# Wangshihu12/colmap-pcd

Measured on AMD Instinct MI355X. Metric: NN queries/sec + BA-iter ms, 10M-pt cloud / 1M 3D feats, higher is better.
Workload: dtype f32 (NN distances) / f64 (association, BA); 1 GPU; M: 10000000-pt 'planes' cloud / 1000000 queries + BA scene 1000 cams / 1000000 pts / 4721253 obs / 900000 lidar terms (OPENCV), the same total at every N; cloud_points=10000000, queries=1000000, queries_this_rank=1000000, parallelism=single GPU

## Files before the change

colmap-pcd_amd/csrc/brick_clip_kernel.h:

```cpp
#pragma once

namespace pcd {

constexpr int kClipNk = 7;
constexpr int kClipRows = 9;
constexpr int kATile = 128;
constexpr int kClipRanges = 10;
#ifdef PCD_ABLATE
constexpr int kAblateClipMath = 0x10000, kAblateBound = 0x20000, kAblateStageA = 0x40000, kAblateSelect = 0x80000;
#else
constexpr int kAblateClipMath = 0, kAblateBound = 0, kAblateStageA = 0, kAblateSelect = 0;
#endif

__device__ __forceinline__ void compare_q1p1(const f32x4 p, const float qx, const float qy, const float qz, double& best) {
  asm("v_mov_b32 v120, %[pw]\n\t"
      "v_sub_f32 v122, %[qx], %[px]\n\tv_sub_f32 v123, %[qy], %[py]\n\tv_sub_f32 v124, %[qz], %[pz]\n\t"
      "v_mul_f32 v122, v122, v122\n\tv_mul_f32 v123, v123, v123\n\tv_mul_f32 v124, v124, v124\n\t"
      "v_add_f32 v122, v122, v123\n\tv_add_f32 v121, v122, v124\n\t"
      "v_min_f64 %[b], %[b], v[120:121]\n\t"
      : [b] "+v"(best)
      : [px] "v"(p.x), [py] "v"(p.y), [pz] "v"(p.z), [pw] "v"(p.w), [qx] "v"(qx), [qy] "v"(qy), [qz] "v"(qz)
      : "v118", "v119", "v120", "v121", "v122", "v123", "v124", "v125", "v126", "v127");
}

template <int NQ, int NP>
__device__ __forceinline__ void compare_step(const f32x4 (&p)[2], const float (&qx)[8], const float (&qy)[8],
                                             const float (&qz)[8], double (&best)[8]) {
  static_assert(NQ >= 1 && NQ <= 8 && (NP == 1 || NP == 2), "1..8 queries, 1 or 2 points");
  constexpr int E = NQ & ~1;
#pragma unroll
  for (int k = 0; k < NP; ++k) {
    if (E >= 4) compare_point4(p[k], qx, qy, qz, best);
    if (E == 8) compare_point4(p[k], qx + 4, qy + 4, qz + 4, best + 4);
    if (E == 2 || E == 6) compare_point2(p[k], qx + (E - 2), qy + (E - 2), qz + (E - 2), best + (E - 2));
  }
  if (NQ & 1) {
    if (NP == 2) compare_query1(p[0], p[1], qx[NQ - 1], qy[NQ - 1], qz[NQ - 1], best[NQ - 1]);
    else compare_q1p1(p[0], qx[NQ - 1], qy[NQ - 1], qz[NQ - 1], best[NQ - 1]);
  }
}

__device__ __forceinline__ float proven_bound_f(const GridParams& g, float qx, float qy, float qz, const int c0[3],
                                                const int c1[3]) {
  const float q[3] = {qx, qy, qz};
  float margin = 3e38f;
#pragma unroll
  for (int d = 0; d < 3; ++d) {
    if (c0[d] > 0) margin = fminf(margin, q[d] - (g.origin[d] + (float)c0[d] * g.h));
    if (c1[d] < g.dims[d]) margin = fminf(margin, (g.origin[d] + (float)c1[d] * g.h) - q[d]);
  }
  if (margin >= 3e38f) return 3e38f;
  margin -= 2.0f * g.slack;
  if (!(margin > 0.0f)) return -1.0f;
  return margin * margin * (1.0f - 1e-5f);
}

constexpr uint64_t span_lanes(int cls) {
  uint64_t m = 0;
  for (int r = 0; r < kClipRows; ++r)
    for (int j = 0; j < 3; ++j)
      if ((j != 1) + (r % 3 != 1) + (r / 3 != 1) == cls) m |= 1ull << (kClipNk * r + 2 * j);
  return m;
}

struct ClipMeta {
  float4 q;
  uint64_t prior;
  uint32_t bnd;
};

__device__ __forceinline__ ClipMeta clip_load_meta(const GridParams& g, const uint4 it, const float4* __restrict__ qsorted,
                                                   const uint64_t* __restrict__ ksorted,
                                                   const uint32_t* __restrict__ cell_start, uint32_t lpos) {
  const int lane = threadIdx.x & 63;
  const int lk = (int)(lpos & 0xFFu), lry = (int)((lpos >> 8) & 0xFFu), lrz = (int)(lpos >> 16);
  ClipMeta m;
  const int cnt = item_count(it);
  m.q = qsorted[it.x + (lane < cnt ? lane : cnt - 1)];
  m.prior = ksorted[it.x + (lane < cnt ? lane : cnt - 1)];
  const int bx = (int)it.y, by = (int)it.z, bz = (int)(it.w & 0x0FFFFFFFu);
  const int yq = by - 1 + lry, zq = bz - 1 + lrz;
  const bool ok = lrz < 3 && yq >= 0 && yq < g.qdims[0] && zq >= 0 && zq < g.qdims[1];
  const int x = min(max(2 * bx - 2 + lk, 0), g.dims[0]);
  const uint32_t v = cell_start[quad_row_base(g, ok ? yq : 0, ok ? zq : 0) + 4u * (uint64_t)x];
  m.bnd = ok ? v : 0u;
  return m;
}

__global__ __launch_bounds__(256, 4) void k_nn_brick_clip(GridParams g, const float4* __restrict__ sorted,
                                                          const uint32_t* __restrict__ cell_start,
                                                          const float4* __restrict__ qsorted,
                                                          const uint64_t* __restrict__ ksorted,
                                                          const uint4* __restrict__ items, NnCounters* __restrict__ ctr,
                                                          uint64_t* __restrict__ keys, uint32_t* __restrict__ fb_list,
                                                          uint32_t* __restrict__ fb_count, int flags) {
  constexpr int G = 8;
  constexpr int NK = kClipNk, NC = kClipNk - 1;
  const int collect_stats = flags & 1;
  const bool no_clip = (flags & 2) != 0;
  __shared__ __attribute__((aligned(16))) float4 s_tile[4][2][kTile];
  __shared__ __attribute__((aligned(16))) float4 s_a[4][kATile];
  const int lane = threadIdx.x & 63;
  const int wave = __builtin_amdgcn_readfirstlane((int)(threadIdx.x >> 6));
  const uint32_t nitems = ctr->nitems;
  const uint32_t nwaves = gridDim.x * 4;
  unsigned long long st_staged = 0, st_pairs = 0, st_groups = 0;
  uint32_t fb_base = 0, fb_left = 0;
  uint32_t lpos;
  {
    const int lrow = (lane * 9363) >> 16, lk = lane - 7 * lrow;
    const int lrz = (lrow * 21846) >> 16, lry = lrow - 3 * lrz;
    lpos = (uint32_t)lk | ((uint32_t)lry << 8) | ((uint32_t)lrz << 16);
    asm volatile("" : "+v"(lpos));
  }
#define PCD_BND(m, e) PCD_RL((m).bnd, (e))

  uint32_t item, item_end, stride;
  if ((gridDim.x & 7u) == 0) {
    const uint32_t cls = blockIdx.x & 7u, per = (nitems + 7u) / 8u;
    stride = (gridDim.x >> 3) * 4;
    item = cls * per + (blockIdx.x >> 3) * 4 + wave;
    item_end = min(nitems, (cls + 1) * per);
  } else {
    stride = nwaves;
    item = blockIdx.x * 4 + wave;
    item_end = nitems;
  }
  if (item >= item_end) return;
  const char* __restrict__ src_bytes = reinterpret_cast<const char*>(sorted);
  float4* const bufA = s_a[wave];
#define PCD_RL(v, r) ((uint32_t)__builtin_amdgcn_readlane((int)(v), (int)(r)))
  struct ARange { uint32_t s, ne; };
  auto issue_a = [&](const ClipMeta& m) -> ARange {
    uint32_t sA = PCD_BND(m, 4 * NK + 2), eA = PCD_BND(m, 4 * NK + 4);
    uint32_t e = 4 * NK + 2;
    if (sA == eA) {
      uint32_t up = (uint32_t)__builtin_amdgcn_update_dpp((int)m.bnd, (int)m.bnd, 0x130, 0xf, 0xf, false);
      up = (uint32_t)__builtin_amdgcn_update_dpp((int)up, (int)up, 0x130, 0xf, 0xf, false);
      const uint32_t size = up - m.bnd;
      const uint64_t occ = __builtin_amdgcn_ballot_w64(size != 0u);
      const uint64_t fc = occ & span_lanes(1), ed = occ & span_lanes(2), co = occ & span_lanes(3);
      const uint64_t pick = fc ? fc : ed ? ed : co;
      if (pick & (pick - 1)) {
        uint32_t key = ((0xFFFFFFu - min(size, 0xFFFFFFu)) << 6) | (uint32_t)lane;
        asm("v_cndmask_b32_e64 %0, -1, %1, %2" : "=v"(key) : "v"(key), "s"(pick));
        e = wave_min_u32(key) & 63u;
      } else if (pick) {
        e = (uint32_t)__builtin_ctzll(pick);
      }
      sA = PCD_RL(m.bnd, e); eA = PCD_RL(m.bnd, e + 2u);
    }
    const uint32_t nA = min(eA - sA, (uint32_t)kATile);
    const uint32_t last = nA ? nA - 1u : 0u;
    const uint32_t i0 = sA + min((uint32_t)lane, last), i1 = sA + min((uint32_t)lane + 64u, last);
    lds_dma16(reinterpret_cast<const float4*>(src_bytes + ((uint64_t)i0 << 4)), bufA);
    lds_dma16(reinterpret_cast<const float4*>(src_bytes + ((uint64_t)i1 << 4)), bufA + 64);
    return ARange{sA, nA | (e << 8)};
  };

  uint4 it0 = items[PCD_UNI(item)];
  ClipMeta m0 = clip_load_meta(g, it0, qsorted, ksorted, cell_start, lpos);
  uint4 it1 = items[PCD_UNI(min(item + stride, item_end - 1))];
  ARange a0 = issue_a(m0);

  for (; item < item_end; item += stride) {
    asm volatile("s_waitcnt vmcnt(0)" ::: "memory");
    __builtin_amdgcn_wave_barrier();
    const ClipMeta m1 = clip_load_meta(g, it1, qsorted, ksorted, cell_start, lpos);
    const uint4 it2 = items[PCD_UNI(min(item + 2 * stride, item_end - 1))];

    const uint32_t cnt = (uint32_t)item_count(it0);
    float qx[G], qy[G], qz[G];
    {
      typedef float f32x3 __attribute__((ext_vector_type(3)));
      const uint32_t qb = lds_addr(s_tile[wave][0]);
      const f32x4 qrec = {m0.q.x, m0.q.y, m0.q.z, m0.q.w};
      f32x3 qv[G];
      asm volatile("ds_write_b128 %9, %8\n\ts_waitcnt lgkmcnt(0)\n\t"
                   "ds_read_b96 %0, %10\n\tds_read_b96 %1, %10 offset:16\n\tds_read_b96 %2, %10 offset:32\n\t"
                   "ds_read_b96 %3, %10 offset:48\n\tds_read_b96 %4, %10 offset:64\n\tds_read_b96 %5, %10 offset:80\n\t"
                   "ds_read_b96 %6, %10 offset:96\n\tds_read_b96 %7, %10 offset:112\n\ts_waitcnt lgkmcnt(0)"
                   : "=&v"(qv[0]), "=&v"(qv[1]), "=&v"(qv[2]), "=&v"(qv[3]), "=&v"(qv[4]), "=&v"(qv[5]), "=&v"(qv[6]), "=&v"(qv[7])
                   : "v"(qrec), "v"(qb + (uint32_t)lane * 16u), "v"(qb)
                   : "memory");
#pragma unroll
      for (int k = 0; k < G; ++k) { qx[k] = qv[k].x; qy[k] = qv[k].y; qz[k] = qv[k].z; }
    }
    const int bx = (int)it0.y, by = (int)it0.z, bz = (int)(it0.w & 0x0FFFFFFFu);
    double best[G];
#pragma unroll
    for (int k = 0; k < G; ++k) best[k] = __builtin_bit_cast(double, kKeyInit);

    const uint32_t sA = a0.s, nA = a0.ne & 0xFFu;
    if (nA > 0 && !(flags & kAblateStageA)) {
      f32x4 pa[2];
      const uint32_t rd = lds_addr(bufA) + lane * 16;
      asm volatile("ds_read_b128 %0, %2\n\tds_read_b128 %1, %2 offset:1024\n\ts_waitcnt lgkmcnt(0)"
                   : "=&v"(pa[0]), "=&v"(pa[1]) : "v"(rd) : "memory");
      if (flags & kAblateCompare) {
        asm volatile("" ::"v"(pa[0]), "v"(pa[1]));
      } else if (nA > 64) {
        switch (cnt) {
          case 1: compare_step<1, 2>(pa, qx, qy, qz, best); break;
          case 2: compare_step<2, 2>(pa, qx, qy, qz, best); break;
          case 3: compare_step<3, 2>(pa, qx, qy, qz, best); break;
          case 4: compare_step<4, 2>(pa, qx, qy, qz, best); break;
          case 5: compare_step<5, 2>(pa, qx, qy, qz, best); break;
          case 6: compare_step<6, 2>(pa, qx, qy, qz, best); break;
          case 7: compare_step<7, 2>(pa, qx, qy, qz, best); break;
          default: compare_step<8, 2>(pa, qx, qy, qz, best); break;
        }
      } else {
        switch (cnt) {
          case 1: compare_step<1, 1>(pa, qx, qy, qz, best); break;
          case 2: compare_step<2, 1>(pa, qx, qy, qz, best); break;
          case 3: compare_step<3, 1>(pa, qx, qy, qz, best); break;
          case 4: compare_step<4, 1>(pa, qx, qy, qz, best); break;
          case 5: compare_step<5, 1>(pa, qx, qy, qz, best); break;
          case 6: compare_step<6, 1>(pa, qx, qy, qz, best); break;
          case 7: compare_step<7, 1>(pa, qx, qy, qz, best); break;
          default: compare_step<8, 1>(pa, qx, qy, qz, best); break;
        }
      }
    }
    const int holder = ((lane & 4) ? 32 : 0) | ((lane & 2) ? 16 : 0) | ((lane & 1) ? 8 : 0);
    uint64_t mine;
    {
      const uint64_t red = __builtin_bit_cast(uint64_t, (flags & kAblateReduce) ? best[0] : wave_min8_key(best));
      mine = ((uint64_t)__shfl((uint32_t)(red >> 32), holder) << 32) | __shfl((uint32_t)red, holder);
      mine = min_u64(mine, m0.prior);
    }
    uint32_t w0 = 0, w1 = 0, w2 = 0;
    if (flags & kAblateClipMath) {
      w0 = w1 = w2 = lane < (int)cnt ? 0x3FFFFu : 0u;
    } else if (lane < (int)cnt) {
      const float d = __uint_as_float((uint32_t)(mine >> 32));
      const float r = __builtin_amdgcn_sqrtf(d) * 1.00001f + ((fabsf(m0.q.x) + fabsf(m0.q.y)) + fabsf(m0.q.z)) * 2.4e-7f + 1e-18f;
      const float tx0 = floorf((m0.q.x - r - g.origin[0]) * g.inv_h), tx1 = floorf((m0.q.x + r - g.origin[0]) * g.inv_h);
      const float ty0 = floorf((m0.q.y - r - g.origin[1]) * g.inv_h * 0.5f), ty1 = floorf((m0.q.y + r - g.origin[1]) * g.inv_h * 0.5f);
      const float tz0 = floorf((m0.q.z - r - g.origin[2]) * g.inv_h * 0.5f), tz1 = floorf((m0.q.z + r - g.origin[2]) * g.inv_h * 0.5f);
      const float fx = (float)(2 * bx - 2), fy = (float)(by - 1), fz = (float)(bz - 1);
      const uint32_t kx0 = (uint32_t)__builtin_amdgcn_fmed3f(tx0 - fx, 0.f, (float)(NC - 1)), kx1 = (uint32_t)__builtin_amdgcn_fmed3f(tx1 - fx, 0.f, (float)(NC - 1));
      const uint32_t ry0 = (uint32_t)__builtin_amdgcn_fmed3f(ty0 - fy, 0.f, 2.f), ry1 = (uint32_t)__builtin_amdgcn_fmed3f(ty1 - fy, 0.f, 2.f);
      const uint32_t rz0 = (uint32_t)__builtin_amdgcn_fmed3f(tz0 - fz, 0.f, 2.f), rz1 = (uint32_t)__builtin_amdgcn_fmed3f(tz1 - fz, 0.f, 2.f);
      const uint32_t xm = (2u << kx1) - (1u << kx0);
      const uint32_t ym = (2u << ry1) - (1u << ry0), zm = (2u << rz1) - (1u << rz0);
      const uint32_t pat = xm * ((ym * 0x421u) & 0x1041u);
      w0 = (zm & 1u) ? pat : 0u; w1 = (zm & 2u) ? pat : 0u; w2 = (zm & 4u) ? pat : 0u;
      if (no_clip) w0 = w1 = w2 = 0x3FFFFu;
    }
#define PCD_OR_SHR(v, ctrl) v |= (uint32_t)__builtin_amdgcn_update_dpp(0, (int)(v), ctrl, 0xf, 0xf, true)
    PCD_OR_SHR(w0, 0x111); PCD_OR_SHR(w1, 0x111); PCD_OR_SHR(w2, 0x111);
    PCD_OR_SHR(w0, 0x112); PCD_OR_SHR(w1, 0x112); PCD_OR_SHR(w2, 0x112);
    PCD_OR_SHR(w0, 0x114); PCD_OR_SHR(w1, 0x114); PCD_OR_SHR(w2, 0x114);
#undef PCD_OR_SHR
    const uint32_t M[3] = {PCD_RL(w0, 7), PCD_RL(w1, 7), PCD_RL(w2, 7)};
    const uint32_t rowA = ((a0.ne >> 8) * 9363u) >> 16;
    const uint32_t bndL = (uint32_t)lane - 7u * rowA < 7u ? min(m0.bnd, sA) : m0.bnd;
    uint32_t rs[kClipRanges], rl[kClipRanges];
#pragma unroll
    for (int r = 0; r < kClipRows; ++r) {
      const uint32_t xm = (M[r / 3] >> (6 * (r % 3))) & 63u;
      const int k0 = xm ? __builtin_ctz(xm) : 0, k1 = xm ? 32 - __builtin_clz(xm) : 0;
      const uint32_t s = PCD_RL(bndL, r * NK + k0), e = PCD_RL(bndL, r * NK + k1);
      rs[r] = s; rl[r] = e - s;
    }
    {
      const uint64_t m54 = (uint64_t)M[0] | ((uint64_t)M[1] << 18) | ((uint64_t)M[2] << 36);
      const uint32_t xm = (uint32_t)(m54 >> (6u * rowA)) & 63u;
      const uint32_t k0 = xm ? (uint32_t)__builtin_ctz(xm) : 0u, k1 = xm ? 32u - (uint32_t)__builtin_clz(xm) : 0u;
      const uint32_t e = PCD_BND(m0, rowA * NK + k1);
      rs[9] = max(PCD_BND(m0, rowA * NK + k0), sA + nA);
      rl[9] = e > rs[9] ? e - rs[9] : 0u;
    }
    uint32_t ro[kClipRanges + 1];
    ro[0] = 0;
#pragma unroll
    for (int i = 0; i < kClipRanges; ++i) ro[i + 1] = ro[i] + ((rl[i] + 3u) & ~3u);
    const uint32_t T = (flags & kAblateTiles) ? 0u : ro[kClipRanges];
    const int ntiles = (int)((T + kTile - 1) / kTile);

    ARange a1;
    if (T > 0) {
      uint32_t dv[kClipRanges];
#pragma unroll
      for (int i = 0; i < kClipRanges; ++i) asm volatile("v_mov_b32 %0, %1" : "=v"(dv[i]) : "s"(rs[i] - ro[i]));
      auto issue_tile = [&](int t) {
        float4* buf = s_tile[wave][t & 1];
        const uint32_t s4 = min((uint32_t)t * kTile + 4u * (uint32_t)lane, T - 4u);
        uint32_t dl = dv[0];
        if (!(flags & kAblateSelect)) {
#define PCD_SEL(o, d) asm("v_cmp_le_u32_e32 vcc, %2, %1\n\tv_cndmask_b32_e32 %0, %0, %3, vcc" : "+v"(dl) : "v"(s4), "s"(o), "v"(d) : "vcc")
        PCD_SEL(ro[1], dv[1]); PCD_SEL(ro[2], dv[2]); PCD_SEL(ro[3], dv[3]); PCD_SEL(ro[4], dv[4]); PCD_SEL(ro[5], dv[5]);
        PCD_SEL(ro[6], dv[6]); PCD_SEL(ro[7], dv[7]); PCD_SEL(ro[8], dv[8]); PCD_SEL(ro[9], dv[9]);
#undef PCD_SEL
        }
        const float4* gp = reinterpret_cast<const float4*>(src_bytes + ((uint64_t)(s4 + dl) << 4));
        if (flags & kAblateNoDma) { asm volatile("" ::"v"(gp)); return; }
        lds_dma16_off<0>(gp, buf);
        lds_dma16_off<16>(gp, buf + 64 - 1);
        lds_dma16_off<32>(gp, buf + 128 - 2);
        lds_dma16_off<48>(gp, buf + 192 - 3);
      };
      issue_tile(0);
      a1 = issue_a(m1);
      auto run_tiles = [&](auto nq_tag) {
        constexpr int NQ = decltype(nq_tag)::value;
        for (int t = 0; t < ntiles; ++t) {
          if (t + 1 < ntiles) {
            issue_tile(t + 1);
            if (t == 0) asm volatile("s_waitcnt vmcnt(6)" ::: "memory");
            else asm volatile("s_waitcnt vmcnt(4)" ::: "memory");
          } else {
            if (t == 0) asm volatile("s_waitcnt vmcnt(2)" ::: "memory");
            else asm volatile("s_waitcnt vmcnt(0)" ::: "memory");
          }
          __builtin_amdgcn_wave_barrier();
          f32x4 p[4];
          const uint32_t rd = lds_addr(s_tile[wave][t & 1]) + lane * 16;
          if (flags & kAblateNoLdsRead) {
#pragma unroll
            for (int k = 0; k < 4; ++k) p[k] = f32x4{(float)lane, (float)t, (float)k, 0.f};
          } else
          asm volatile("ds_read_b128 %0, %4\n\tds_read_b128 %1, %4 offset:1024\n\t"
                       "ds_read_b128 %2, %4 offset:2048\n\tds_read_b128 %3, %4 offset:3072\n\t"
                       "s_waitcnt lgkmcnt(0)"
                       : "=&v"(p[0]), "=&v"(p[1]), "=&v"(p[2]), "=&v"(p[3])
                       : "v"(rd)
                       : "memory");
          if (flags & kAblateCompare) {
#pragma unroll
            for (int k = 0; k < 4; ++k) asm volatile("" ::"v"(p[k]));
          } else {
            compare_tile<NQ>(p, qx, qy, qz, best);
          }
        }
      };
      switch (cnt) {
        case 1: run_tiles(std::integral_constant<int, 1>{}); break;
        case 2: run_tiles(std::integral_constant<int, 2>{}); break;
        case 3: run_tiles(std::integral_constant<int, 3>{}); break;
        case 4: run_tiles(std::integral_constant<int, 4>{}); break;
        case 5: run_tiles(std::integral_constant<int, 5>{}); break;
        case 6: run_tiles(std::integral_constant<int, 6>{}); break;
        case 7: run_tiles(std::integral_constant<int, 7>{}); break;
        default: run_tiles(std::integral_constant<int, 8>{}); break;
      }
      const uint64_t red = __builtin_bit_cast(uint64_t, (flags & kAblateReduce) ? best[0] : wave_min8_key(best));
      mine = min_u64(mine, ((uint64_t)__shfl((uint32_t)(red >> 32), holder) << 32) | __shfl((uint32_t)red, holder));
    } else {
      a1 = issue_a(m1);
    }
    bool unproven = false;
    if (lane < (int)cnt) {
      const uint32_t my_qi = __float_as_uint(m0.q.w);
      const int c0[3] = {max(2 * bx - 2, 0), max(2 * by - 2, 0), max(2 * bz - 2, 0)};
      const int c1[3] = {min(2 * bx + 4, g.dims[0]), min(2 * by + 4, g.dims[1]), min(2 * bz + 4, g.dims[2])};
      const float bound = (flags & kAblateBound) ? 3e38f : proven_bound_f(g, m0.q.x, m0.q.y, m0.q.z, c0, c1);
      unproven = !(__uint_as_float((uint32_t)(mine >> 32)) < bound) && !(flags & kAblateFallback);
      keys[my_qi] = unproven ? mine : finalized_key(mine);
    }
    const unsigned long long um = __ballot(unproven);
    if (um) {
      const uint32_t k = (uint32_t)__popcll(um);
      if (k > fb_left) {
        if (lane < (int)fb_left) fb_list[fb_base + lane] = 0xFFFFFFFFu;
        uint32_t nb = 0;
        if (lane == 0) nb = atomicAdd(fb_count, (uint32_t)kFbChunk);
        fb_base = (uint32_t)__builtin_amdgcn_readfirstlane((int)nb);
        fb_left = kFbChunk;
      }
      if (unproven) fb_list[fb_base + __builtin_amdgcn_mbcnt_hi((uint32_t)(um >> 32), __builtin_amdgcn_mbcnt_lo((uint32_t)um, 0u))] = __float_as_uint(m0.q.w);
      fb_base += k;
      fb_left -= k;
    }
    if (collect_stats) {
      const uint32_t slots = (nA > 64 ? 128u : nA ? 64u : 0u) + (uint32_t)ntiles * kTile;
      st_staged += nA + T; st_pairs += (unsigned long long)slots * cnt; st_groups += 1;
    }
    it0 = it1; it1 = it2; m0 = m1; a0 = a1;
  }
  asm volatile("s_waitcnt vmcnt(0)" ::: "memory");
  if (lane < (int)fb_left) fb_list[fb_base + lane] = 0xFFFFFFFFu;
  if (collect_stats && lane == 0) {
    atomicAdd(&ctr->staged_points, st_staged);
    atomicAdd(&ctr->pair_evals, st_pairs);
    atomicAdd(&ctr->brick_groups, st_groups);
  }
#undef PCD_BND
#undef PCD_RL
}

}
```

colmap-pcd_amd/csrc/nn.hip:

```cpp
#include <atomic>
#include <cfloat>

#include "cloud.h"
#include "grid.h"
#include "prim.h"
#include "scratch.h"

namespace pcd {

void free_query_scratch(QueryScratch* s) { delete s; }

constexpr uint64_t kKeyInit = (uint64_t)0x7F7FFFFFu << 32;
constexpr uint64_t kSmallBatch = 65536;

struct BrickParams {
  int B, R;
  int Bx;
  int nb[3];
  uint32_t nbricks;
};

constexpr int kBrickCells = 2, kBrickCellsX = 2, kBrickHalo = 2;

static BrickParams make_bricks(const GridParams& g) {
// ... 631 lines not shown
      const uint32_t cn_ = (cn);                                                                                      \
      const uint32_t last = cn_ ? cn_ - 1u : 0u;                   \
      const uint32_t id = (cf) + ((uint32_t)lane < last ? (uint32_t)lane : last);                                     \
      const float4 lo = *reinterpret_cast<const float4*>(aabb + 8 * (size_t)id);             \
      const float4 hi = *reinterpret_cast<const float4*>(aabb + 8 * (size_t)id + 4);       \
           \
                      \
      const float px = __builtin_amdgcn_fmed3f(qx, lo.x, lo.w), pyc = __builtin_amdgcn_fmed3f(qy, lo.y, hi.x),        \
                  pz = __builtin_amdgcn_fmed3f(qz, lo.z, hi.y);                                                       \
      const float lbv = l2_simple3(qx, qy, qz, px, pyc, pz);                                                          \
      cur_lb = (uint32_t)lane < cn_ ? lbv : INFINITY;                                                                 \
      rs = __float_as_uint(hi.z); rn = __float_as_uint(hi.w);                                                         \
      cur_m = __ballot(cur_lb <= best_d);                                                                             \
    }
    PCD_FB_EXPAND(py.root_first, py.root_count);
    while (true) {
      ++q_steps;
      unsigned long long m = cur_m & __ballot(cur_lb <= best_d);
      if (m == 0) {
        if (lev == top) break;
        ++lev;
        cur_lb = s_lb[wave][lev - 2][lane];
        const uint32_t pr = s_rng[wave][lev - 2][lane];
        rs = pr & (kMaxPyrRecords - 1u); rn = (pr >> 26) + 1u;
        const unsigned long long pm = s_mask[wave][lev - 2];
        cur_m = ((unsigned long long)(uint32_t)__builtin_amdgcn_readfirstlane((int)(pm >> 32)) << 32) |
                (uint32_t)__builtin_amdgcn_readfirstlane((int)pm);
        continue;
      }
      const int sl = wave_argmin_u32(__float_as_uint(cur_lb), m);
      m &= ~(1ull << sl);
      cur_m = m;
      if (lev == 1) {
        const uint32_t s0 = (uint32_t)__builtin_amdgcn_readlane((int)rs, sl), n0 = (uint32_t)__builtin_amdgcn_readlane((int)rn, sl);
        for (uint32_t base = 0; base < n0; base += 128) {
          float4 p[2];
#pragma unroll
          for (int k = 0; k < 2; ++k) {
            const uint32_t gi = base + k * 64 + lane;
            p[k] = sorted[s0 + (gi < n0 ? gi : n0 - 1)];
          }
#pragma unroll
          for (int k = 0; k < 2; ++k) {
            const float d = l2_simple3(qx, qy, qz, p[k].x, p[k].y, p[k].z);
            lane_best = min_key_f64(lane_best, __builtin_bit_cast(double, make_key(d, __float_as_uint(p[k].w))));
          }
        }
        st_pts += n0;
        ++q_leaves;
        best = wave_min_u64(__builtin_bit_cast(uint64_t, lane_best));
        best_d = __uint_as_float((uint32_t)(best >> 32));
        unsigned long long mb = m & __ballot(cur_lb <= best_d);
        if (mb) {
          cur_m = m & ~mb;
          while (mb) {
            uint32_t a[4], c[4];
            uint32_t cmax = 0;
#pragma unroll
            for (int k = 0; k < 4; ++k) {
              const int r = mb ? __ffsll((long long)mb) - 1 : -1;
              mb &= mb - 1;
              a[k] = r >= 0 ? (uint32_t)__builtin_amdgcn_readlane((int)rs, r) : a[0];
              c[k] = r >= 0 ? (uint32_t)__builtin_amdgcn_readlane((int)rn, r) : 0u;
              cmax = c[k] > cmax ? c[k] : cmax;
              st_pts += c[k];
              q_leaves += r >= 0 ? 1 : 0;
            }
            for (uint32_t base = 0; base < cmax; base += 64) {
              float4 p[4];
              const uint32_t gi = base + lane;
#pragma unroll
              for (int k = 0; k < 4; ++k) p[k] = sorted[a[k] + (gi < c[k] ? gi : (c[k] ? c[k] - 1 : 0u))];
#pragma unroll
              for (int k = 0; k < 4; ++k) {
                const float d = l2_simple3(qx, qy, qz, p[k].x, p[k].y, p[k].z);
                lane_best = min_key_f64(lane_best, __builtin_bit_cast(double, make_key(d, __float_as_uint(p[k].w))));
              }
            }
          }
          best = wave_min_u64(__builtin_bit_cast(uint64_t, lane_best));
          best_d = __uint_as_float((uint32_t)(best >> 32));
        }
      } else {
        s_lb[wave][lev - 2][lane] = cur_lb;
        s_rng[wave][lev - 2][lane] = rs | ((rn - 1u) << 26);
        if (lane == 0) s_mask[wave][lev - 2] = cur_m;
        const uint32_t cf = (uint32_t)__builtin_amdgcn_readlane((int)rs, sl), cn = (uint32_t)__builtin_amdgcn_readlane((int)rn, sl);
        --lev;
        PCD_FB_EXPAND(cf, cn);
      }
    }
#undef PCD_FB_EXPAND
    if (lane == 0) keys[qi] = finalized_key(best);
    st_q += 1;
    st_steps += q_steps; st_leaves += q_leaves;
    st_max_steps = q_steps > st_max_steps ? q_steps : st_max_steps;
    st_max_leaves = q_leaves > st_max_leaves ? q_leaves : st_max_leaves;
  }
  if (collect_stats) {
    __shared__ unsigned long long s_st[4];
    __shared__ unsigned int s_mx[2];
    if (threadIdx.x < 4) s_st[threadIdx.x] = 0;
    if (threadIdx.x < 2) s_mx[threadIdx.x] = 0;
    __syncthreads();
    if (lane == 0) {
      atomicAdd(&s_st[0], st_pts); atomicAdd(&s_st[1], st_q); atomicAdd(&s_st[2], st_steps); atomicAdd(&s_st[3], st_leaves);
      atomicMax(&s_mx[0], st_max_steps); atomicMax(&s_mx[1], st_max_leaves);
    }
    __syncthreads();
    if (threadIdx.x == 0 && s_st[1]) {
      atomicAdd(&ctr->fallback_points, s_st[0]);
      atomicAdd(&ctr->pair_evals, s_st[0]);
      atomicAdd(&ctr->fallback_queries, s_st[1]);
      atomicAdd(&ctr->fb_steps, s_st[2]); atomicAdd(&ctr->fb_leaves, s_st[3]);
      atomicMax(&ctr->fb_max_steps, s_mx[0]); atomicMax(&ctr->fb_max_leaves, s_mx[1]);
    }
  }
}

constexpr unsigned g_fb_max_blocks = 16384;
struct FbQueries {
  const float4* qf4;
  FbFused fused;
  const uint32_t *list, *list_count;
};
template <int FUSED>
static void launch_fallback(const pcd_cloud* c, const float4* seeds, const FbQueries& src, uint64_t n, uint64_t* keys,
                            NnCounters* ctr, int collect_stats, hipStream_t s) {
  hipLaunchKernelGGL(k_nn_fallback<FUSED>, dim3((unsigned)std::min<uint64_t>(div_up(n, 4), g_fb_max_blocks)), dim3(256), 0,
                     s, c->grid, c->pyr, c->sorted.p, c->cell_start.p, c->blk_aabb.p, seeds, src.qf4, src.list,
                     src.list_count, src.list_count ? 0u : (uint32_t)n, keys, ctr, collect_stats, src.fused);
}
static std::atomic<int> g_collect_stats{0};
#ifdef PCD_ABLATE
static const int g_brick_blocks_per_cu = std::getenv("PCD_BRICK_BLOCKS") ? std::atoi(std::getenv("PCD_BRICK_BLOCKS")) : PCD_BRICK_MINWAVES;
#else
constexpr int g_brick_blocks_per_cu = PCD_BRICK_MINWAVES;
#endif
static std::atomic<int> g_nn_kernel{0};
static std::atomic<int> g_bk_sort{0};

static pcd_status brick_slots(pcd_cloud* c, QueryScratch* sc, const BrickParams& b, hipStream_t s) {
  if (sc->bk_slot.p && sc->bk_nslots == b.nbricks) return PCD_OK;
  PCD_TRY(sc->bk_slot.reserve((size_t)b.nbricks / 32 + 1));
  DevBuf<uint32_t> flag;
  PCD_TRY(flag.reserve((size_t)b.nbricks + 1));
  hipLaunchKernelGGL(k_brick_occupied, dim3(div_up(b.nbricks, 256)), dim3(256), 0, s, c->grid, b, c->cell_start.p, flag.p);
  hipLaunchKernelGGL(k_brick_bitmap, dim3(div_up(div_up(b.nbricks, 32), 256)), dim3(256), 0, s, flag.p, b.nbricks, sc->bk_slot.p);
  PCD_HIP_TRY(hipStreamSynchronize(s));
  sc->bk_nslots = b.nbricks;
  return PCD_OK;
}

__global__ void k_seed_init(GridParams g, int sdx, int sdy, int sdz, float4* __restrict__ seeds, float4* __restrict__ qf4,
                            uint64_t* __restrict__ keys) {
  const uint64_t i = blockIdx.x * (uint64_t)blockDim.x + threadIdx.x;
  if (i >= (uint64_t)sdx * sdy * sdz) return;
  const int x = (int)(i % sdx), y = (int)((i / sdx) % sdy), z = (int)(i / ((uint64_t)sdx * sdy));
  seeds[i] = make_float4(INFINITY, INFINITY, INFINITY, 0.f);
  const float cx = 0.5f * (float)(8 * x + min(8 * x + 8, g.dims[0])), cy = 0.5f * (float)(8 * y + min(8 * y + 8, g.dims[1])),
              cz = 0.5f * (float)(8 * z + min(8 * z + 8, g.dims[2]));
  qf4[i] = make_float4(g.origin[0] + cx * g.h, g.origin[1] + cy * g.h, g.origin[2] + cz * g.h, 1.f);
  keys[i] = kKeyInit;
}
__global__ void k_seed_gather(const uint64_t* __restrict__ keys, uint64_t n, ShardIndex si, const float4* __restrict__ pts4,
                              float4* __restrict__ seeds) {
  const uint64_t i = blockIdx.x * (uint64_t)blockDim.x + threadIdx.x;
  if (i >= n) return;
  const uint64_t k = keys[i];
  const uint64_t row = k == PCD_KEY_NONE ? ~0ull : shard_local_row(si, (uint32_t)k);
  if (row == ~0ull) return;
  const float4 p = pts4[row];
  seeds[i] = make_float4(p.x, p.y, p.z, __uint_as_float((uint32_t)k));
}
static pcd_status fb_seed_table(pcd_cloud* c, QueryScratch* sc, hipStream_t s) {
  if (sc->fb_seed_ok) return PCD_OK;
  const PyramidParams& py = c->pyr;
  const uint64_t n = (uint64_t)py.seed_dims[0] * py.seed_dims[1] * py.seed_dims[2];
  DevBuf<float4> qf4;
  DevBuf<uint64_t> keys;
  DevBuf<float4>& seeds = sc->fb_seed;
  PCD_TRY(seeds.reserve(n));
  PCD_TRY(qf4.reserve(n));
  PCD_TRY(keys.reserve(n));
  hipLaunchKernelGGL(k_seed_init, dim3(div_up(n, 256)), dim3(256), 0, s, c->grid, py.seed_dims[0], py.seed_dims[1],
                     py.seed_dims[2], seeds.p, qf4.p, keys.p);
  launch_fallback<0>(c, seeds.p, {qf4.p}, n, keys.p, nullptr, 0, s);
  hipLaunchKernelGGL(k_seed_gather, dim3(div_up(n, 256)), dim3(256), 0, s, keys.p, n, c->shard_index(), c->pts4.p, seeds.p);
  PCD_HIP_TRY(hipGetLastError());
  PCD_HIP_TRY(hipStreamSynchronize(s));
  sc->fb_seed_ok = true;
  return PCD_OK;
}

static pcd_status counters_ready(QueryScratch* sc, hipStream_t s) {
  if (sc->counters.p) return PCD_OK;
  PCD_TRY(sc->counters.reserve(2));
  PCD_HIP_TRY(hipMemsetAsync(sc->counters.p, 0, 2 * sizeof(NnCounters), s));
  sc->ctr_cur = 0;
  sc->ctr_next_clean = true;
  return PCD_OK;
}
enum class CtrUse { kAlternate, kClear, kClearForStats };
static pcd_status take_counters(QueryScratch* sc, CtrUse use, int collect_stats, hipStream_t s, NnCounters** ctr,
                                NnCounters** ctr_next = nullptr) {
  PCD_TRY(counters_ready(sc, s));
  const bool clean = use == CtrUse::kAlternate ? sc->ctr_next_clean : use == CtrUse::kClearForStats && !collect_stats;
  if (use == CtrUse::kAlternate) {
    sc->ctr_cur = 1 - sc->ctr_cur;
    sc->ctr_next_clean = false;
  }
  *ctr = sc->counters.p + sc->ctr_cur;
  if (ctr_next) *ctr_next = sc->counters.p + (1 - sc->ctr_cur);
  if (!clean) PCD_HIP_TRY(hipMemsetAsync(*ctr, 0, sizeof(NnCounters), s));
  return PCD_OK;
}
static void counters_left_clean(QueryScratch* sc) { sc->ctr_next_clean = true; }

static void launch_prepare(const NnCall& call, uint64_t Q, float4* qf4, uint64_t* d_keys, hipStream_t s) {
  ScopedKernelTimer t("nn_prepare", s);
  with_prep_mode(call.prep, [&](auto mode) {
    hipLaunchKernelGGL(k_prepare<decltype(mode)::value>, dim3(div_up(Q, 256)), dim3(256), 0, s, call.pa, Q, qf4, d_keys);
  });
}
static void launch_finalize(uint64_t Q, uint64_t* d_keys, hipStream_t s) {
  ScopedKernelTimer t("nn_finalize", s);
  hipLaunchKernelGGL(k_finalize_keys, dim3(div_up(Q, 256)), dim3(256), 0, s, d_keys, Q);
}
static void launch_bruteforce(const pcd_cloud* c, const float4* qf4, uint64_t Q, uint64_t* d_keys, hipStream_t s) {
  ScopedKernelTimer t("nn_bruteforce", s);
  const unsigned qblocks = div_up(Q, 256);
  unsigned chunks = std::max(1u, std::min<unsigned>(div_up(c->n, 4096), 2048u / std::max(1u, qblocks)));
  chunks = std::min(chunks, 65535u);
  const uint64_t chunk = ((c->n + chunks - 1) / chunks + 1023) / 1024 * 1024;
  chunks = div_up(c->n, chunk);
  hipLaunchKernelGGL(k_nn_bruteforce, dim3(qblocks, chunks), dim3(256), 0, s, c->pts4.p, c->n, c->index_base,
                     c->index_stride, c->row_index.p, qf4, Q, chunk, d_keys);
}

constexpr int kGroup = 8;
static pcd_status run_grid(pcd_cloud* c, QueryScratch* sc, uint64_t Q, uint64_t* d_keys, hipStream_t s, const NnCall& call) {
  const uint64_t* carried_keys = call.prep != kPrepPlain ? d_keys : nullptr;
  const GridParams& g = c->grid;
  const int nn_kernel = g_nn_kernel.load(), bk_sort = g_bk_sort.load(), collect_stats = g_collect_stats.load();
  const BrickParams b = make_bricks(g);
  PCD_TRY(sc->qsorted.reserve(Q));
  PCD_TRY(sc->ksorted.reserve(Q));
  const size_t fb_cap = Q + Q / 8 + 8 + (size_t)256 * g_brick_blocks_per_cu * 4 * kFbChunk +
                        (size_t)2048 * 4 * 64;
  PCD_TRY(sc->fb_list.reserve(fb_cap));
  PCD_TRY(sc->bk_keys.reserve(2 * Q));
  PCD_TRY(sc->bk_vals.reserve(2 * Q));
  PCD_TRY(sc->bk_item.reserve(div_up(Q, kBkTile) + 1));
  PCD_TRY(sc->items.reserve(Q + 1));
  PCD_TRY(counters_ready(sc, s));
  PCD_TRY(brick_slots(c, sc, b, s));
  uint32_t shift = 8;
  while ((((uint64_t)b.nbricks + (1u << shift) - 1) >> shift) > 2304 && shift < 16) ++shift;
  const uint32_t ncoarse = std::max<uint32_t>(1u, (uint32_t)(((uint64_t)b.nbricks + (1u << shift) - 1) >> shift));
  const bool counting = (1u << shift) <= kBkMaxFine && ncoarse <= kBkMaxCoarse && bk_sort == 0;
  NnCounters *ctr, *ctr_next;
  PCD_TRY(take_counters(sc, counting ? CtrUse::kAlternate : CtrUse::kClear, collect_stats, s, &ctr, &ctr_next));
  if (counting) {
    ScopedKernelTimer t("nn_brick_bookkeeping", s);
    const uint32_t nrounds = div_up(Q, kBkTileQ), rounds = div_up(nrounds, kBkMaxRanges), nranges = div_up(nrounds, rounds);
    PCD_TRY(sc->bk_chist.reserve(3 * (size_t)kBkMaxCoarse + 3));
    PCD_TRY(sc->bk_hmat.reserve((size_t)nranges * ncoarse));
    uint32_t *ctot = sc->bk_chist.p, *cstart = ctot + kBkMaxCoarse + 1, *bitems = cstart + kBkMaxCoarse + 1;
    uint32_t* qslot = sc->bk_keys.p;
    uint2* ppair = reinterpret_cast<uint2*>(sc->bk_vals.p);
    with_prep_mode(call.prep, [&](auto mode) {
      hipLaunchKernelGGL(k_bk_slots<decltype(mode)::value>, dim3(nranges), dim3(1024), 0, s, call.pa, (uint32_t)Q, rounds,
                         g, b, sc->bk_slot.p, shift, ncoarse, sc->qf4.p, d_keys, qslot, sc->bk_hmat.p, sc->fb_list.p, ctr,
                         ctr_next);
    });
    hipLaunchKernelGGL(k_bk_colscan, dim3(div_up(ncoarse, 64)), dim3(1024), 0, s, sc->bk_hmat.p, nranges, ncoarse, ctot);
    hipLaunchKernelGGL(k_bk_scatter, dim3(nranges), dim3(1024), 0, s, qslot, (uint32_t)Q, rounds, shift, ncoarse, ctot,
                       sc->bk_hmat.p, cstart, ppair, ctr);
    hipLaunchKernelGGL(k_bk_count<kGroup>, dim3(ncoarse), dim3(256), 0, s, shift, cstart, ppair, bitems);
    hipLaunchKernelGGL(k_bk_emit<kGroup>, dim3(ncoarse), dim3(256), (3u * (1u << shift) + 2u) * sizeof(uint32_t), s,
                       sc->qf4.p, carried_keys, g, b, shift, cstart, ppair, bitems, sc->items.p, sc->qsorted.p, sc->ksorted.p, ctr);
  } else {
    launch_prepare(call, Q, sc->qf4.p, d_keys, s);
    ScopedKernelTimer t("nn_brick_bookkeeping", s);
    uint32_t *k0 = sc->bk_keys.p, *k1 = sc->bk_keys.p + Q, *v0 = sc->bk_vals.p, *v1 = sc->bk_vals.p + Q;
    hipLaunchKernelGGL(k_brick_keys, dim3(div_up(Q, 256)), dim3(256), 0, s, sc->qf4.p, Q, g, b, k0, v0);
    unsigned end_bit = 1;
    while (end_bit < 32 && ((uint64_t)1 << end_bit) <= (uint64_t)b.nbricks + 1) ++end_bit;
#ifndef PCD_SORT_MERGE_LIMIT
#define PCD_SORT_MERGE_LIMIT 262144
#endif
    using SortCfg = rocprim::radix_sort_config<rocprim::default_config, rocprim::default_config,
                                               rocprim::default_config, PCD_SORT_MERGE_LIMIT>;
    PCD_TRY(sort_pairs<SortCfg>(sc->tmp, k0, k1, v0, v1, (unsigned)Q, 0u, end_bit, s));
    const unsigned ntiles = div_up(Q, kBkTile);
    hipLaunchKernelGGL(k_brick_tile_count<kGroup>, dim3(ntiles), dim3(256), 0, s, k1, (uint32_t)Q, b.nbricks, sc->bk_item.p);
    hipLaunchKernelGGL(k_brick_emit<kGroup>, dim3(ntiles), dim3(256), 0, s, k1, v1, sc->bk_item.p, sc->qf4.p, carried_keys,
                       (uint32_t)Q, b.nbricks, (uint32_t)b.nb[0], (uint32_t)b.nb[1], sc->items.p, sc->qsorted.p,
                       sc->ksorted.p, sc->fb_list.p, ctr);
  }
  {
    ScopedKernelTimer t("nn_brick", s);
    const unsigned blocks = (unsigned)std::min<uint64_t>(div_up(div_up(Q, kGroup), 4) + 1, 256 * (uint64_t)g_brick_blocks_per_cu);
    const int fl = (collect_stats & ~2) | (nn_kernel == 1 ? 2 : 0);
    hipLaunchKernelGGL(k_nn_brick_clip, dim3(blocks), dim3(256), 0, s, g, c->sorted.p, c->cell_start.p, sc->qsorted.p,
                       sc->ksorted.p, sc->items.p, ctr, d_keys, sc->fb_list.p, &ctr->fb_count, fl);
  }
  {
    ScopedKernelTimer t("nn_fallback", s);
    PCD_TRY(sc->fb_dense.reserve(Q));
    hipLaunchKernelGGL(k_fb_compact, dim3(div_up(fb_cap, kFbcThreads * kFbcPer)), dim3(kFbcThreads), 0, s, sc->fb_list.p,
                       &ctr->fb_count, sc->fb_dense.p, &ctr->pad[0]);
    launch_fallback<0>(c, sc->fb_seed.p, {sc->qf4.p, {}, sc->fb_dense.p, &ctr->pad[0]}, Q, d_keys, ctr, collect_stats, s);
  }
  PCD_HIP_TRY(hipGetLastError());
  if (counting) counters_left_clean(sc);
  return PCD_OK;
}

enum class NnPath { kEmptyCloud, kBruteForce, kOneLaunch, kPrepareWalk, kGrid };
static pcd_status choose_path(bool empty_cloud, int algo, uint64_t Q, int prep, NnPath* path) {
  const NnPath walk = prep == kPrepRefine ? NnPath::kPrepareWalk : NnPath::kOneLaunch;
  if (empty_cloud) *path = NnPath::kEmptyCloud;
  else if (algo == PCD_NN_BRUTEFORCE) *path = NnPath::kBruteForce;
  else if (algo == PCD_NN_FALLBACK_ONLY) *path = walk;
  else if (algo == PCD_NN_AUTO) *path = Q <= kSmallBatch ? walk : NnPath::kGrid;
  else if (algo == PCD_NN_GRID) *path = NnPath::kGrid;
  else {
    set_error("unknown nn algo %d", algo);
    return PCD_ERR_INVALID;
  }
  return PCD_OK;
}

static pcd_status nn_device(pcd_cloud* c, const NnCall& call, uint64_t Q, int algo, uint64_t* d_keys, hipStream_t s) {
  QueryScratch* sc = scratch_of(c);
  if (Q == 0) return PCD_OK;
  PCD_REQUIRE(Q < 0xFFFFFFF0ull, "more than 2^32 queries in one call");
  NnPath path;
  PCD_TRY(choose_path(c->m == 0, algo, Q, call.prep, &path));
  const int collect_stats = g_collect_stats.load();
  NnCounters* ctr;
  switch (path) {
    case NnPath::kEmptyCloud:
    case NnPath::kBruteForce:
      PCD_TRY(sc->qf4.reserve(Q));
      launch_prepare(call, Q, sc->qf4.p, d_keys, s);
      if (path == NnPath::kBruteForce) launch_bruteforce(c, sc->qf4.p, Q, d_keys, s);
      launch_finalize(Q, d_keys, s);
      break;
    case NnPath::kOneLaunch: {
      PCD_TRY(fb_seed_table(c, sc, s));
      PCD_TRY(take_counters(sc, CtrUse::kClearForStats, collect_stats, s, &ctr));
      ScopedKernelTimer t("nn_fallback", s);
      const FbQueries src{nullptr, FbFused{call.pa.q, call.pa.max_range, call.pa.mr_count, call.pa.fixed_range}};
      if (call.prep == kPrepBounded) launch_fallback<2>(c, sc->fb_seed.p, src, Q, d_keys, ctr, collect_stats, s);
      else launch_fallback<1>(c, sc->fb_seed.p, src, Q, d_keys, ctr, collect_stats, s);
      break;
    }
    case NnPath::kPrepareWalk: {
      PCD_TRY(fb_seed_table(c, sc, s));
      PCD_TRY(sc->qf4.reserve(Q));
      launch_prepare(call, Q, sc->qf4.p, d_keys, s);
      PCD_TRY(take_counters(sc, CtrUse::kClear, collect_stats, s, &ctr));
      ScopedKernelTimer t("nn_fallback", s);
      launch_fallback<0>(c, sc->fb_seed.p, {sc->qf4.p}, Q, d_keys, ctr, collect_stats, s);
      break;
    }
    case NnPath::kGrid:
      PCD_TRY(fb_seed_table(c, sc, s));
      PCD_TRY(sc->qf4.reserve(Q));
      PCD_TRY(run_grid(c, sc, Q, d_keys, s, call));
      break;
  }
  PCD_HIP_TRY(hipGetLastError());
  return PCD_OK;
}

static NnCall make_call(int prep, const pcd_cloud* c, const double* d_q, const uint8_t* d_skip = nullptr,
                        const double* d_max_range = nullptr, uint64_t mr_count = 0, double fixed_range = 0.0) {
  const BoxF box{c->bb_lo[0], c->bb_lo[1], c->bb_lo[2], c->bb_hi[0], c->bb_hi[1], c->bb_hi[2]};
  return {prep, {d_q, d_skip, box, d_max_range, mr_count, fixed_range}};
}

pcd_status nn_query_device_internal(pcd_cloud* c, const double* d_q, uint64_t Q, int algo, uint64_t* d_keys,
                                    hipStream_t s) {
  return nn_device(c, make_call(kPrepPlain, c, d_q), Q, algo, d_keys, s);
}
pcd_status nn_query_bounded_internal(pcd_cloud* c, const double* d_q, uint64_t Q, const double* d_max_range,
                                     uint64_t mr_count, double fixed_range, uint64_t* d_keys, hipStream_t s) {
  return nn_device(c, make_call(kPrepBounded, c, d_q, nullptr, d_max_range, mr_count, fixed_range), Q, PCD_NN_AUTO, d_keys, s);
}

}

using namespace pcd;

extern "C" {

pcd_status pcd_nn_query_device(pcd_cloud* c, const double* d_q_xyz, uint64_t Q, int algo, uint64_t* d_keys,
                               void* stream) {
  PCD_REQUIRE(c, "null cloud");
  PCD_REQUIRE(Q == 0 || (d_q_xyz && d_keys), "null pointer");
  PCD_REFUSE_CAPTURE(stream);
  PCD_HIP_TRY(hipSetDevice(c->device));
  return nn_device(c, make_call(kPrepPlain, c, d_q_xyz), Q, algo, d_keys, (hipStream_t)stream);
}

pcd_status pcd_nn_refine_device(pcd_cloud* c, const double* d_q_xyz, uint64_t Q, const uint8_t* d_skip,
                                uint64_t* d_keys, void* stream) {
  PCD_REQUIRE(c, "null cloud");
  PCD_REQUIRE(Q == 0 || (d_q_xyz && d_keys), "null pointer");
  PCD_REFUSE_CAPTURE(stream);
  PCD_HIP_TRY(hipSetDevice(c->device));
  return nn_device(c, make_call(kPrepRefine, c, d_q_xyz, d_skip), Q, PCD_NN_AUTO, d_keys, (hipStream_t)stream);
}

pcd_status pcd_nn_query_algo(pcd_cloud* c, const double* q_xyz, uint64_t Q, int algo, uint32_t* idx, float* sqdist,
                             uint8_t* found) {
  PCD_REQUIRE(c, "null cloud");
  PCD_REQUIRE(Q == 0 || (q_xyz && idx && sqdist && found), "null pointer");
  if (Q == 0) return PCD_OK;
  PCD_HIP_TRY(hipSetDevice(c->device));
  QueryScratch* sc = scratch_of(c);
  hipStream_t s = nullptr;
  PCD_TRY(sc->d_q.reserve(3 * Q));
  PCD_TRY(sc->keys.reserve(Q));
  PCD_TRY(sc->d_idx.reserve(Q));
  PCD_TRY(sc->d_sq.reserve(Q));
  PCD_TRY(sc->d_found.reserve(Q));
  PCD_HIP_TRY(hipMemcpyAsync(sc->d_q.p, q_xyz, 3 * Q * sizeof(double), hipMemcpyHostToDevice, s));
  PCD_TRY(nn_device(c, make_call(kPrepPlain, c, sc->d_q.p), Q, algo, sc->keys.p, s));
  hipLaunchKernelGGL(k_unpack_keys, dim3(div_up(Q, 256)), dim3(256), 0, s, sc->keys.p, Q, sc->d_idx.p, sc->d_sq.p,
                     sc->d_found.p);
  PCD_HIP_TRY(hipMemcpyAsync(idx, sc->d_idx.p, Q * sizeof(uint32_t), hipMemcpyDeviceToHost, s));
  PCD_HIP_TRY(hipMemcpyAsync(sqdist, sc->d_sq.p, Q * sizeof(float), hipMemcpyDeviceToHost, s));
  PCD_HIP_TRY(hipMemcpyAsync(found, sc->d_found.p, Q * sizeof(uint8_t), hipMemcpyDeviceToHost, s));
  PCD_HIP_TRY(hipStreamSynchronize(s));
  return PCD_OK;
}

pcd_status pcd_nn_query(pcd_cloud* c, const double* q_xyz, uint64_t Q, uint32_t* idx, float* sqdist, uint8_t* found) {
  return pcd_nn_query_algo(c, q_xyz, Q, PCD_NN_AUTO, idx, sqdist, found);
}

pcd_status pcd_nn_last_stats(pcd_cloud* c, pcd_nn_stats* st) {
  PCD_REQUIRE(c && st, "null pointer");
  std::memset(st, 0, sizeof *st);
  if (!c->scratch || !c->scratch->counters.p) return PCD_OK;
  PCD_HIP_TRY(hipSetDevice(c->device));
  PCD_HIP_TRY(hipDeviceSynchronize());
  NnCounters h;
  PCD_HIP_TRY(hipMemcpy(&h, c->scratch->counters.p + c->scratch->ctr_cur, sizeof h, hipMemcpyDeviceToHost));
  st->brick_groups = h.brick_groups;
  st->staged_points = h.staged_points;
  st->fallback_queries = h.fallback_queries;
  st->fallback_points = h.fallback_points;
  st->pair_evals = h.pair_evals;
  static const bool print_walks = std::getenv("PCD_FB_STATS") != nullptr;
  if (print_walks)
    std::fprintf(stderr, "[pcd] fallback walk: %llu queries, %.1f steps / %.1f leaf scans per query, max %u / %u\n",
                 (unsigned long long)h.fallback_queries, h.fallback_queries ? (double)h.fb_steps / h.fallback_queries : 0.0,
                 h.fallback_queries ? (double)h.fb_leaves / h.fallback_queries : 0.0, h.fb_max_steps, h.fb_max_leaves);
  return PCD_OK;
}

pcd_status pcd_nn_set_search(int kernel) {
  if (kernel < 0) return PCD_OK;
  PCD_REQUIRE(kernel <= 1, "kernel must be 0 (clipped brick kernel) or 1 (the same with the clip off); there is no separate "
                           "whole-region kernel: the clip-off switch, pcd_nn_set_search(1), is the A/B reference");
  g_nn_kernel = kernel;
  return PCD_OK;
}

pcd_status pcd_nn_set_bookkeeping(int radix_sort) {
  g_bk_sort = radix_sort ? 1 : 0;
  return PCD_OK;
}

pcd_status pcd_nn_set_tuning(int brick_cells, int halo_cells, int collect_stats) {
  if ((brick_cells != 0 && brick_cells != kBrickCells) || (halo_cells >= 0 && halo_cells != kBrickHalo)) {
    set_error("pcd_nn_set_tuning: the brick geometry is fixed at %d cells with a halo of %d (asked for %d / %d)",
              kBrickCells, kBrickHalo, brick_cells, halo_cells);
    return PCD_ERR_UNSUPPORTED;
  }
#ifdef PCD_ABLATE
  g_collect_stats = collect_stats;
#else
  g_collect_stats = collect_stats & 1;
#endif
  return PCD_OK;
}

}
```

Before: 807.3 million queries/s.

## Skip per-query tile comparisons outside each query's clip window in brick kernel

Adds a per-query tile loop used when a group holds at least three queries. Each query gets a 63-bit ownership mask of the cells its search radius touches. Each lane gets the set of tiles that overlap its hull cell, and two ballots give a per-tile active-query mask, so only those queries run the point comparisons. This cuts wasted distance evaluations for queries whose clipped region misses a tile. In exchange it adds ballot and select work per tile, swaps compile-time-unrolled NQ specialisation for runtime branches per query, and moves the proven-bound computation ahead of the tile loop.

```diff
diff --git a/colmap-pcd_amd/csrc/brick_clip_kernel.h b/colmap-pcd_amd/csrc/brick_clip_kernel.h
--- a/colmap-pcd_amd/csrc/brick_clip_kernel.h
+++ b/colmap-pcd_amd/csrc/brick_clip_kernel.h
@@ -7,10 +7,15 @@
 constexpr int kATile = 128;
 constexpr int kClipRanges = 10;
 #ifdef PCD_ABLATE
-constexpr int kAblateClipMath = 0x10000, kAblateBound = 0x20000, kAblateStageA = 0x40000, kAblateSelect = 0x80000;
+constexpr int kAblateClipMath = 0x10000, kAblateBound = 0x20000, kAblateStageA = 0x40000, kAblateSelect = 0x80000,
+              kAblateQueryTest = 0x100000;
 #else
-constexpr int kAblateClipMath = 0, kAblateBound = 0, kAblateStageA = 0, kAblateSelect = 0;
+constexpr int kAblateClipMath = 0, kAblateBound = 0, kAblateStageA = 0, kAblateSelect = 0, kAblateQueryTest = 0;
 #endif
+#ifndef PCD_QCLIP_MIN
+#define PCD_QCLIP_MIN 3
+#endif
+constexpr int kQClipMin = PCD_QCLIP_MIN;
 
 __device__ __forceinline__ void compare_q1p1(const f32x4 p, const float qx, const float qy, const float qz, double& best) {
   asm("v_mov_b32 v120, %[pw]\n\t"
@@ -231,8 +236,10 @@
       mine = min_u64(mine, m0.prior);
     }
     uint32_t w0 = 0, w1 = 0, w2 = 0;
+    uint64_t own = 0;
     if (flags & kAblateClipMath) {
       w0 = w1 = w2 = lane < (int)cnt ? 0x3FFFFu : 0u;
+      own = lane < (int)cnt ? ~0ull : 0ull;
     } else if (lane < (int)cnt) {
       const float d = __uint_as_float((uint32_t)(mine >> 32));
       const float r = __builtin_amdgcn_sqrtf(d) * 1.00001f + ((fabsf(m0.q.x) + fabsf(m0.q.y)) + fabsf(m0.q.z)) * 2.4e-7f + 1e-18f;
@@ -247,6 +254,8 @@
       const uint32_t ym = (2u << ry1) - (1u << ry0), zm = (2u << rz1) - (1u << rz0);
       const uint32_t pat = xm * ((ym * 0x421u) & 0x1041u);
       w0 = (zm & 1u) ? pat : 0u; w1 = (zm & 2u) ? pat : 0u; w2 = (zm & 4u) ? pat : 0u;
+      const uint64_t pat7 = xm * ((ym * 0x1041u) & 0x4081u);
+      own = ((zm & 1u) ? pat7 : 0ull) | ((zm & 2u) ? pat7 << 21 : 0ull) | ((zm & 4u) ? pat7 << 42 : 0ull);
       if (no_clip) w0 = w1 = w2 = 0x3FFFFu;
     }
 #define PCD_OR_SHR(v, ctrl) v |= (uint32_t)__builtin_amdgcn_update_dpp(0, (int)(v), ctrl, 0xf, 0xf, true)
@@ -280,7 +289,16 @@
     const uint32_t T = (flags & kAblateTiles) ? 0u : ro[kClipRanges];
     const int ntiles = (int)((T + kTile - 1) / kTile);
 
+    uint32_t my_qi = __float_as_uint(m0.q.w);
+    float bound;
+    {
+      const int c0[3] = {max(2 * bx - 2, 0), max(2 * by - 2, 0), max(2 * bz - 2, 0)};
+      const int c1[3] = {min(2 * bx + 4, g.dims[0]), min(2 * by + 4, g.dims[1]), min(2 * bz + 4, g.dims[2])};
+      bound = (flags & kAblateBound) ? 3e38f : proven_bound_f(g, m0.q.x, m0.q.y, m0.q.z, c0, c1);
+      asm volatile("" : "+v"(bound), "+v"(my_qi));
+    }
     ARange a1;
+    uint32_t tile_queries = (uint32_t)ntiles * cnt;
     if (T > 0) {
       uint32_t dv[kClipRanges];
 #pragma unroll
@@ -304,30 +322,33 @@
       };
       issue_tile(0);
       a1 = issue_a(m1);
+      auto fetch_tile = [&](int t, f32x4 (&p)[4]) {
+        if (t + 1 < ntiles) {
+          issue_tile(t + 1);
+          if (t == 0) asm volatile("s_waitcnt vmcnt(6)" ::: "memory");
+          else asm volatile("s_waitcnt vmcnt(4)" ::: "memory");
+        } else {
+          if (t == 0) asm volatile("s_waitcnt vmcnt(2)" ::: "memory");
+          else asm volatile("s_waitcnt vmcnt(0)" ::: "memory");
+        }
+        __builtin_amdgcn_wave_barrier();
+        const uint32_t rd = lds_addr(s_tile[wave][t & 1]) + lane * 16;
+        if (flags & kAblateNoLdsRead) {
+#pragma unroll
+          for (int k = 0; k < 4; ++k) p[k] = f32x4{(float)lane, (float)t, (float)k, 0.f};
+        } else
+        asm volatile("ds_read_b128 %0, %4\n\tds_read_b128 %1, %4 offset:1024\n\t"
+                     "ds_read_b128 %2, %4 offset:2048\n\tds_read_b128 %3, %4 offset:3072\n\t"
+                     "s_waitcnt lgkmcnt(0)"
+                     : "=&v"(p[0]), "=&v"(p[1]), "=&v"(p[2]), "=&v"(p[3])
+                     : "v"(rd)
+                     : "memory");
+      };
       auto run_tiles = [&](auto nq_tag) {
         constexpr int NQ = decltype(nq_tag)::value;
         for (int t = 0; t < ntiles; ++t) {
-          if (t + 1 < ntiles) {
-            issue_tile(t + 1);
-            if (t == 0) asm volatile("s_waitcnt vmcnt(6)" ::: "memory");
-            else asm volatile("s_waitcnt vmcnt(4)" ::: "memory");
-          } else {
-            if (t == 0) asm volatile("s_waitcnt vmcnt(2)" ::: "memory");
-            else asm volatile("s_waitcnt vmcnt(0)" ::: "memory");
-          }
-          __builtin_amdgcn_wave_barrier();
           f32x4 p[4];
-          const uint32_t rd = lds_addr(s_tile[wave][t & 1]) + lane * 16;
-          if (flags & kAblateNoLdsRead) {
-#pragma unroll
-            for (int k = 0; k < 4; ++k) p[k] = f32x4{(float)lane, (float)t, (float)k, 0.f};
-          } else
-          asm volatile("ds_read_b128 %0, %4\n\tds_read_b128 %1, %4 offset:1024\n\t"
-                       "ds_read_b128 %2, %4 offset:2048\n\tds_read_b128 %3, %4 offset:3072\n\t"
-                       "s_waitcnt lgkmcnt(0)"
-                       : "=&v"(p[0]), "=&v"(p[1]), "=&v"(p[2]), "=&v"(p[3])
-                       : "v"(rd)
-                       : "memory");
+          fetch_tile(t, p);
           if (flags & kAblateCompare) {
 #pragma unroll
             for (int k = 0; k < 4; ++k) asm volatile("" ::"v"(p[k]));
@@ -336,6 +357,60 @@
           }
         }
       };
+      auto run_tiles_per_query = [&]() -> uint32_t {
+        uint32_t lp = lpos;
+        asm volatile("" : "+v"(lp));
+        const uint32_t lk = lp & 0xFFu, lry = (lp >> 8) & 0xFFu, lrz = lp >> 16;
+        const uint32_t lrow = lry + 3u * lrz;
+        const uint32_t up = (uint32_t)__builtin_amdgcn_update_dpp((int)m0.bnd, (int)m0.bnd, 0x130, 0xf, 0xf, false);
+        const uint64_t m54 = (uint64_t)M[0] | ((uint64_t)M[1] << 18) | ((uint64_t)M[2] << 36);
+        const uint32_t mrow = (uint32_t)(m54 >> (6u * lrow)) & 63u;
+        const bool hull = lk < (uint32_t)NC && lrz < 3u && (mrow >> lk) != 0u && (mrow & ((2u << lk) - 1u)) != 0u;
+        const bool rest = lrow == rowA && (uint32_t)lane >= (a0.ne >> 8);
+        auto vsel = [](uint32_t a, uint32_t b, uint64_t m) {
+          uint32_t r;
+          asm("v_cndmask_b32_e64 %0, %1, %2, %3" : "=v"(r) : "v"(a), "v"(b), "s"(m));
+          return r;
+        };
+        const uint64_t y1 = __builtin_amdgcn_ballot_w64(lry == 1u), y2 = __builtin_amdgcn_ballot_w64(lry == 2u);
+        uint32_t dl = vsel(vsel(dv[0], dv[1], y1), dv[2], y2);
+        dl = vsel(dl, vsel(vsel(dv[3], dv[4], y1), dv[5], y2), __builtin_amdgcn_ballot_w64(lrz == 1u));
+        dl = vsel(dl, vsel(vsel(dv[6], dv[7], y1), dv[8], y2), __builtin_amdgcn_ballot_w64(lrz == 2u));
+        dl = vsel(dl, dv[9], __builtin_amdgcn_ballot_w64(rest));
+        const uint32_t lo = rest ? max(m0.bnd, sA + nA) : m0.bnd;
+        const bool any = hull && up > lo;
+        const uint32_t tlo = min((lo - dl) >> 8, 31u), thi = min((up - 1u - dl) >> 8, 31u);
+        const uint32_t tmask = any ? (2u << thi) - (1u << tlo) : 0u;
+        const uint32_t own_lo = (uint32_t)own, own_hi = (uint32_t)(own >> 32);
+        uint32_t compared = 0;
+        for (int t = 0; t < ntiles; ++t) {
+          uint32_t act;
+          if (flags & kAblateQueryTest) {
+            act = (1u << cnt) - 1u;
+          } else {
+            const uint64_t occ = __builtin_amdgcn_ballot_w64((tmask & (1u << min(t, 31))) != 0u);
+            act = (uint32_t)__builtin_amdgcn_ballot_w64(((own_lo & (uint32_t)occ) | (own_hi & (uint32_t)(occ >> 32))) != 0u);
+          }
+          compared += (uint32_t)__builtin_popcount(act);
+          f32x4 p[4];
+          fetch_tile(t, p);
+          if (flags & kAblateCompare) {
+#pragma unroll
+            for (int k = 0; k < 4; ++k) asm volatile("" ::"v"(p[k]));
+          } else {
+#pragma unroll
+            for (int k = 0; k < G; ++k)
+              if (act & (1u << k)) {
+                compare_query1(p[0], p[1], qx[k], qy[k], qz[k], best[k]);
+                compare_query1(p[2], p[3], qx[k], qy[k], qz[k], best[k]);
+              }
+          }
+        }
+        return compared;
+      };
+      if (cnt >= (uint32_t)kQClipMin && !(flags & 6)) {
+        tile_queries = run_tiles_per_query();
+      } else
       switch (cnt) {
         case 1: run_tiles(std::integral_constant<int, 1>{}); break;
         case 2: run_tiles(std::integral_constant<int, 2>{}); break;
@@ -353,10 +428,6 @@
     }
     bool unproven = false;
     if (lane < (int)cnt) {
-      const uint32_t my_qi = __float_as_uint(m0.q.w);
-      const int c0[3] = {max(2 * bx - 2, 0), max(2 * by - 2, 0), max(2 * bz - 2, 0)};
-      const int c1[3] = {min(2 * bx + 4, g.dims[0]), min(2 * by + 4, g.dims[1]), min(2 * bz + 4, g.dims[2])};
-      const float bound = (flags & kAblateBound) ? 3e38f : proven_bound_f(g, m0.q.x, m0.q.y, m0.q.z, c0, c1);
       unproven = !(__uint_as_float((uint32_t)(mine >> 32)) < bound) && !(flags & kAblateFallback);
       keys[my_qi] = unproven ? mine : finalized_key(mine);
     }
@@ -370,13 +441,13 @@
         fb_base = (uint32_t)__builtin_amdgcn_readfirstlane((int)nb);
         fb_left = kFbChunk;
       }
-      if (unproven) fb_list[fb_base + __builtin_amdgcn_mbcnt_hi((uint32_t)(um >> 32), __builtin_amdgcn_mbcnt_lo((uint32_t)um, 0u))] = __float_as_uint(m0.q.w);
+      if (unproven) fb_list[fb_base + __builtin_amdgcn_mbcnt_hi((uint32_t)(um >> 32), __builtin_amdgcn_mbcnt_lo((uint32_t)um, 0u))] = my_qi;
       fb_base += k;
       fb_left -= k;
     }
     if (collect_stats) {
-      const uint32_t slots = (nA > 64 ? 128u : nA ? 64u : 0u) + (uint32_t)ntiles * kTile;
-      st_staged += nA + T; st_pairs += (unsigned long long)slots * cnt; st_groups += 1;
+      const uint32_t slots = (nA > 64 ? 128u : nA ? 64u : 0u) * cnt + tile_queries * kTile;
+      st_staged += nA + T; st_pairs += slots; st_groups += 1;
     }
     it0 = it1; it1 = it2; m0 = m1; a0 = a1;
   }
diff --git a/colmap-pcd_amd/csrc/nn.hip b/colmap-pcd_amd/csrc/nn.hip
--- a/colmap-pcd_amd/csrc/nn.hip
+++ b/colmap-pcd_amd/csrc/nn.hip
@@ -957,7 +957,7 @@
   {
     ScopedKernelTimer t("nn_brick", s);
     const unsigned blocks = (unsigned)std::min<uint64_t>(div_up(div_up(Q, kGroup), 4) + 1, 256 * (uint64_t)g_brick_blocks_per_cu);
-    const int fl = (collect_stats & ~2) | (nn_kernel == 1 ? 2 : 0);
+    const int fl = (collect_stats & ~6) | (nn_kernel == 1 ? 2 : nn_kernel == 3 ? 4 : 0);
     hipLaunchKernelGGL(k_nn_brick_clip, dim3(blocks), dim3(256), 0, s, g, c->sorted.p, c->cell_start.p, sc->qsorted.p,
                        sc->ksorted.p, sc->items.p, ctr, d_keys, sc->fb_list.p, &ctr->fb_count, fl);
   }
@@ -1122,8 +1122,10 @@
 
 pcd_status pcd_nn_set_search(int kernel) {
   if (kernel < 0) return PCD_OK;
-  PCD_REQUIRE(kernel <= 1, "kernel must be 0 (clipped brick kernel) or 1 (the same with the clip off); there is no separate "
-                           "whole-region kernel: the clip-off switch, pcd_nn_set_search(1), is the A/B reference");
+  PCD_REQUIRE(kernel <= 1 || kernel == 3,
+              "kernel must be 0 (clipped brick kernel), 1 (the same with the clip off) or 3 (the same without the per-query "
+              "clip of the tile loop); there is no separate whole-region kernel (the retired value 2): the clip-off "
+              "switch, pcd_nn_set_search(1), is the A/B reference");
   g_nn_kernel = kernel;
   return PCD_OK;
 }
```

New measurement: 814.3 million queries/s (median of 6 runs). Within noise of the previous version (+0.9%).
